# xiangli0608/Creating-2D-laser-slam-from-scratch

Measured on AMD Instinct MI355X. Metric: scan-matches/sec (1081-beam vs 2000x2000 grid), higher is better.
Workload: dtype u8

## Files before the change

### creating-2d-laser-slam-from-scratch_amd/api.py

```python
from __future__ import annotations

import ctypes as C
import os
import sys
import math
import weakref

import numpy as np

from . import build as _build

LSLAM_OK = 0
ERRORS = {
    -1: "LSLAM_ERR_INVALID_ARGUMENT",
    -2: "LSLAM_ERR_NO_DEVICE",
    -3: "LSLAM_ERR_INDEX_OUT_OF_RANGE",
    -4: "LSLAM_ERR_PROBABILITY_SEARCH",
    -5: "LSLAM_ERR_NO_BEST_POSE",
    -6: "LSLAM_ERR_HIP",
    -7: "LSLAM_ERR_SMEAR_DEVIATION",
    -8: "LSLAM_ERR_UNSUPPORTED",
}


# ... 774 lines not shown
    L.lslam_profile_only.argtypes = [vp, C.c_char_p]
    L.lslam_profile_reset.argtypes = [vp]
    L.lslam_profile_read.argtypes = [vp, vp, i32]
    L.lslam_matcher_config_defaults.argtypes = [C.POINTER(MatcherConfig)]
    L.lslam_matcher_config_defaults.restype = None
    L.lslam_matcher_create.argtypes = [vp, C.POINTER(MatcherConfig), C.POINTER(LaserParams), C.POINTER(vp)]
    L.lslam_debug_reduce_lds_bytes.argtypes = [C.POINTER(MatcherConfig), i32, C.POINTER(i32 * 3)]
    L.lslam_debug_reduce_lds_bytes.restype = i32
    L.lslam_matcher_destroy.argtypes = [vp]
    L.lslam_matcher_destroy.restype = None
    L.lslam_matcher_num_beams.argtypes = [vp]
    L.lslam_matcher_grid_info.argtypes = [vp, vp, vp]
    L.lslam_matcher_get_grid_u8.argtypes = [vp, vp]
    L.lslam_matcher_get_kernel_u8.argtypes = [vp, vp]
    L.lslam_matcher_set_grid_u8.argtypes = [vp, vp, vp]
    L.lslam_matcher_set_grid_u8_dev.argtypes = [vp, vp, vp]
    L.lslam_matcher_grid_dev_ptr.restype = vp
    L.lslam_matcher_grid_dev_ptr.argtypes = [vp]
    L.lslam_sensor_pose_from_robot.argtypes = [C.POINTER(LaserParams), vp, vp]
    L.lslam_sensor_pose_from_robot.restype = None
    L.lslam_robot_pose_from_sensor.argtypes = [C.POINTER(LaserParams), vp, vp]
    L.lslam_robot_pose_from_sensor.restype = None
    L.lslam_matcher_set_base_scans.argtypes = [vp, i32, vp, i32, vp, vp]
    L.lslam_matcher_match_scan.argtypes = [vp, i32, vp, i32, vp, vp, vp, i32, i32, vp]
    L.lslam_matcher_match_batch.argtypes = [vp, i32, vp, i32, vp, i32, i32, vp]
    L.lslam_matcher_match_batch_dev_f32.argtypes = [vp, i32, vp, i32, vp, i32, i32, vp]
    L.lslam_matcher_match_batch_dev_f64.argtypes = [vp, i32, vp, i32, vp, i32, i32, vp]
    L.lslam_matcher_debug_lookup_table.argtypes = [vp, vp, vp, dbl, dbl, dbl, vp, C.POINTER(i32)]
    L.lslam_matcher_debug_coarse_sums.argtypes = [vp, vp, vp, vp, C.POINTER(i32), C.POINTER(i32),
                                                  C.POINTER(i32), i32]
    L.lslam_matcher_debug_coarse_sums_batch.argtypes = [vp, i32, vp, i32, vp, vp]
    L.lslam_matcher_debug_fine_sums_batch.argtypes = [vp, i32, vp, i32, vp, vp, vp, C.POINTER(i32), C.POINTER(i32), C.POINTER(i32)]
    L.lslam_matcher_debug_valid_mask.argtypes = [vp, vp, vp, vp, vp]
    L.lslam_frontend_create.argtypes = [vp, i32, dbl, dbl, dbl, C.POINTER(vp)]
    L.lslam_frontend_destroy.argtypes = [vp]
    L.lslam_frontend_destroy.restype = None
    L.lslam_frontend_reset.argtypes = [vp]
    L.lslam_frontend_process.argtypes = [vp, vp, i32, vp, C.POINTER(i32), vp, vp, C.POINTER(dbl)]
    L.lslam_frontend_running_scans.argtypes = [vp]
    L.lslam_frontend_config_defaults.argtypes = [C.POINTER(FrontEndConfig)]
    L.lslam_frontend_config_defaults.restype = None
    L.lslam_frontend_create_ex.argtypes = [vp, C.POINTER(FrontEndConfig), C.POINTER(vp)]
    L.lslam_frontend_process_stamped.argtypes = [vp, vp, i32, vp, dbl, C.POINTER(i32), vp, vp, C.POINTER(dbl)]
    L.lslam_frontend_num_scans.argtypes = [vp]
    L.lslam_frontend_scan_pose.argtypes = [vp, i32, vp]
    L.lslam_frontend_stats.argtypes = [vp, vp]
    L.lslam_frontend_process_many.argtypes = [vp, i32, vp, i32, vp, vp, vp, vp, vp, vp]
    L.lslam_frontend_lookahead_stats.argtypes = [vp, vp]
    L.lslam_frontend_spec_chain_stats.argtypes = [vp, vp]
    L.lslam_debug_frontend_anchor_row.argtypes = [vp, C.c_int, vp]
    L.lslam_occgrid_create_from_scans.argtypes = [vp, C.POINTER(LaserParams), i32, vp, i32, vp, dbl, C.POINTER(vp)]
    L.lslam_occgrid_destroy.argtypes = [vp]
    L.lslam_occgrid_destroy.restype = None
    L.lslam_occgrid_info.argtypes = [vp, vp, vp, C.POINTER(dbl)]
    L.lslam_occgrid_read_u8.argtypes = [vp, vp]
    L.lslam_occgrid_read_ros_i8.argtypes = [vp, vp]
    L.lslam_occgrid_scan_bounds.argtypes = [vp, C.POINTER(LaserParams), i32, vp, i32, vp, vp]
    L.lslam_occgrid_create_partial.argtypes = [vp, C.POINTER(LaserParams), i32, vp, i32, vp, dbl, vp, C.POINTER(vp)]
    L.lslam_occgrid_counter_words.argtypes = [vp, C.POINTER(C.c_size_t)]
    L.lslam_occgrid_export_counters.argtypes = [vp, vp, i32]
    L.lslam_occgrid_import_counters.argtypes = [vp, vp, i32, i32]
    L.lslam_occgrid_counters_dev_ptr.restype = vp
    L.lslam_occgrid_counters_dev_ptr.argtypes = [vp]
    L.lslam_occgrid_ray_cast.argtypes = [vp, i32, vp, vp, dbl, vp]
    L.lslam_occgrid_ray_cast_dev.argtypes = [vp, i32, vp, vp, dbl, vp]
    L.lslam_occgrid_ray_cast_scans.argtypes = [vp, C.POINTER(LaserParams), i32, vp, dbl, vp, i32]
# ... 486 lines not shown
        nx, ny, na = C.c_int(), C.c_int(), C.c_int()
        self.ctx.check(self.L.lslam_matcher_debug_coarse_sums(self.h, r.ctypes.data, p.ctypes.data, None,
                                                              C.byref(nx), C.byref(ny), C.byref(na), 0))
        out = np.zeros((ny.value, nx.value, na.value), dtype=np.int32)
        self.ctx.check(self.L.lslam_matcher_debug_coarse_sums(self.h, r.ctypes.data, p.ctypes.data, out.ctypes.data,
                                                              C.byref(nx), C.byref(ny), C.byref(na),
                                                              int(force_generic)))
        return out

    def coarse_sums_batch(self, ranges, sensor_poses) -> np.ndarray:
        r, p = _f64(ranges), _f64(sensor_poses)
        n = r.shape[0]
        nx, ny, na = C.c_int(), C.c_int(), C.c_int()
        self.ctx.check(self.L.lslam_matcher_debug_coarse_sums(self.h, r.ctypes.data, p.ctypes.data, None,
                                                              C.byref(nx), C.byref(ny), C.byref(na), 0))
        out = np.zeros((n, ny.value, nx.value, na.value), dtype=np.int32)
        self.ctx.check(self.L.lslam_matcher_debug_coarse_sums_batch(self.h, n, r.ctypes.data, r.shape[1], p.ctypes.data,
                                                                    out.ctypes.data))
        return out

    def fine_sums_batch(self, ranges, sensor_poses):
        r, p = _f64(ranges), _f64(sensor_poses)
        n = r.shape[0]
        nx, ny, na = C.c_int(), C.c_int(), C.c_int()
        self.ctx.check(self.L.lslam_matcher_debug_fine_sums_batch(self.h, n, r.ctypes.data, r.shape[1], p.ctypes.data, None, None,
                                                                  C.byref(nx), C.byref(ny), C.byref(na)))
        out = np.zeros((n, ny.value, nx.value, na.value), dtype=np.int32)
        centers = np.zeros((n, 3))
        self.ctx.check(self.L.lslam_matcher_debug_fine_sums_batch(self.h, n, r.ctypes.data, r.shape[1], p.ctypes.data,
                                                                  centers.ctypes.data, out.ctypes.data, C.byref(nx), C.byref(ny),
                                                                  C.byref(na)))
        return out, centers

    def valid_mask(self, ranges, sensor_pose, viewpoint) -> np.ndarray:
        r, p, v = _f64(ranges), _f64(sensor_pose), _f64(viewpoint)
        out = np.zeros(self.num_beams, dtype=np.uint8)
        self.ctx.check(self.L.lslam_matcher_debug_valid_mask(self.h, r.ctypes.data, p.ctypes.data, v.ctypes.data,
                                                             out.ctypes.data))
        return out


class ScanCache:

    PENALIZE, REFINE, QUERY_TAKES_RESULT_POSE = 1, 2, 4

    def __init__(self, ctx: Context, laser: LaserParams):
        self.ctx, self.L = ctx, ctx.L
        h = C.c_void_p()
        ctx.check(self.L.lslam_scan_cache_create(ctx.h, C.byref(laser), C.byref(h)))
        self.h = h
        ctx._adopt(self)

    def close(self):
        if getattr(self, "h", None):
            self.L.lslam_scan_cache_destroy(self.h)
            self.h = None

    def __del__(self):
        try:
            if sys.is_finalizing():
                return
            self.close()
        except Exception:
            pass

    def put(self, scan_id: int, ranges):
# ... 1189 lines not shown
```

### creating-2d-laser-slam-from-scratch_amd/csrc/karto_math.hpp

```cpp
#pragma once

#include <hip/hip_runtime.h>

#include <climits>
#include <cmath>
#include <cstdint>

namespace lslam {

#define LSLAM_HD __host__ __device__ __forceinline__

constexpr double kPi = 3.14159265358979323846;
constexpr double k2Pi = 6.28318530717958647692;
constexpr double kPi180 = 0.01745329251994329577;
constexpr double kTol = 1e-06;
constexpr int32_t kInvalidScan = INT_MAX;
constexpr double kMaxVariance = 500.0;
constexpr double kDistPenaltyGain = 0.2;
constexpr double kAnglePenaltyGain = 0.2;
constexpr int kOccupied = 100;

LSLAM_HD double kround(double v) { return v >= 0.0 ? floor(v + 0.5) : ceil(v - 0.5); }
LSLAM_HD double ksq(double v) { return v * v; }
LSLAM_HD bool double_equal(double a, double b) {
  double d = a - b;
  return d < 0.0 ? d >= -kTol : d <= kTol;
}
LSLAM_HD double normalize_angle(double angle) {
  while (angle < -kPi) {
    if (angle < -k2Pi)
      angle += (uint32_t)(angle / -k2Pi) * k2Pi;
    else
      angle += k2Pi;
  }
  while (angle > kPi) {
    if (angle > k2Pi)
      angle -= (uint32_t)(angle / k2Pi) * k2Pi;
    else
      angle -= k2Pi;
  }
  return angle;
}
LSLAM_HD double normalize_angle_difference(double minuend, double subtrahend) {
  while (minuend - subtrahend < -kPi) minuend += k2Pi;
  while (minuend - subtrahend > kPi) minuend -= k2Pi;
  return minuend;
}
LSLAM_HD int world_to_grid(double w, double offset, double scale) {
  return (int)kround((w - offset) * scale);
}
LSLAM_HD int lattice_count(double offset, double resolution) {
  return (int)(uint32_t)(kround(offset * 2.0 / resolution) + 1);
}

struct Rot2 {
  double m00, m01, m02, m10, m11, m12;
};
LSLAM_HD Rot2 rot_z(double radians) {
  const double x = 0.0, y = 0.0, z = 1.0;
  double c = cos(radians), s = sin(radians), omc = 1.0 - c;
  double xyM = x * y * omc, xzM = x * z * omc, yzM = y * z * omc;
  double xS = x * s, yS = y * s, zS = z * s;
  Rot2 r;
  r.m00 = x * x * omc + c;
  r.m01 = xyM - zS;
  r.m02 = xzM + yS;
  r.m10 = xyM + zS;
  r.m11 = y * y * omc + c;
  r.m12 = yzM - xS;
  return r;
}
LSLAM_HD Rot2 rot_identity() { return Rot2{1.0, 0.0, 0.0, 0.0, 1.0, 0.0}; }
LSLAM_HD void rot_apply(const Rot2& r, double x, double y, double h, double& ox, double& oy) {
  ox = r.m00 * x + r.m01 * y + r.m02 * h;
  oy = r.m10 * x + r.m11 * y + r.m12 * h;
}

struct SensorXform {
  Rot2 rot, inv;
  double tx, ty, th;
};
LSLAM_HD SensorXform sensor_xform(double px, double py, double ph) {
  SensorXform t;
  if (px == 0.0 && py == 0.0 && ph == 0.0) {
    t.rot = rot_identity();
    t.inv = rot_identity();
    t.tx = t.ty = t.th = 0.0;
    return t;
  }
  t.rot = rot_z(ph - 0.0);
  t.inv = rot_z(0.0 - ph);
  t.tx = px;
  t.ty = py;
  t.th = ph - 0.0;
  return t;
}

LSLAM_HD void beam_world_point(double sx, double sy, double sh, double min_angle, double ang_res,
                               uint32_t beam, double r, double& px, double& py) {
  double angle = sh + min_angle + beam * ang_res;
#if defined(__HIP_DEVICE_COMPILE__)
  double sn, cs;
  sincos(angle, &sn, &cs);
  px = sx + (r * cs);
  py = sy + (r * sn);
#else
  px = sx + (r * cos(angle));
  py = sy + (r * sin(angle));
#endif
}

LSLAM_HD void lookup_cell(double lx, double ly, double cosine, double sine, double off_x, double off_y,
                          double scale, int& gx, int& gy) {
  double ox = cosine * lx - sine * ly;
  double oy = sine * lx + cosine * ly;
  gx = world_to_grid(ox + off_x, off_x, scale);
  gy = world_to_grid(oy + off_y, off_y, scale);
}
LSLAM_HD int kround_i32(double v) {
  const int i = (int)(fabs(v) + 0.5);
  return v < 0.0 ? -i : i;
}
LSLAM_HD void lookup_cell_i32(double lx, double ly, double cosine, double sine, double off_x, double off_y,
                              double scale, int& gx, int& gy) {
// ... 111 lines not shown
```

### creating-2d-laser-slam-from-scratch_amd/csrc/scan_matcher.hip

```cpp
#include <algorithm>
#include <atomic>
#include <chrono>
#include <cmath>
#include <cstdlib>
#include <cstring>
#include <type_traits>
#include <vector>

#include "common.hpp"
#include "karto_math.hpp"

using namespace lslam;

#if defined(LSLAM_EXP_SERIAL_PRIO)
#define LSLAM_SERIAL_BEGIN() __builtin_amdgcn_s_setprio(3)
#define LSLAM_SERIAL_END() __builtin_amdgcn_s_setprio(0)
#else
#define LSLAM_SERIAL_BEGIN()
#define LSLAM_SERIAL_END()
#endif

namespace {

LSLAM_STAMP_TABLE(g_sm_stamps)
// ... 31 lines not shown
  if (sc.fast_div) {
    const double q = a * sc.inv_denom;
    return __builtin_fma(__builtin_fma(-q, d, a), sc.inv_denom, q);
  }
  return a / d;
}

constexpr int kTilePad = 512;
constexpr int kTileYOff = 32;
constexpr int kRowZero = 64;
constexpr int kMaxBeamsPerLane = 32;
constexpr int kOccMinScans = 8;
constexpr int kTileMinWaves = 2048;
constexpr int kPipeMinChunk = 256;
constexpr int kMaxGridSide = 32768;

struct Lattice {
  double center[3];
  int gx[kMaxLattice], gy[kMaxLattice];
  int step_x, step_y;
  int status, active;
};

struct CoarseOut {
  double mean[3];
  double cov[9];
  double best;
  int status;
  int expand;
  int flags;
  int pad;
};

__device__ __forceinline__ void pass_setup_wave(int s, int lane, const Geom& g, const PassCfg& pc,
                                                const double* center, int active, Lattice* lat,
                                                double2* cossin, int want_step);

struct PoseArg {
  double v[3];
};
template <typename RT>
__device__ __forceinline__ void scan_prep_block(const RT* __restrict__ ranges, int stride, double sx, double sy, double sh,
                                                const Geom& g, double2* __restrict__ local, double2* __restrict__ world,
                                                const PassCfg& setup_pc, Lattice* setup_lat, double2* setup_cossin,
                                                int setup_step, int bx, int nbx, int s) {
  const int nt = (int)blockDim.x;
  int b = bx * nt + threadIdx.x;
  LSLAM_PHASE_CLOCK(pck);
  __shared__ SensorXform s_t;
  __shared__ double s_h;
  if (local && threadIdx.x == 0) {
    LSLAM_SERIAL_BEGIN();
    s_t = sensor_xform(sx, sy, sh);
    s_h = normalize_angle(0.0 - s_t.th);
    LSLAM_SERIAL_END();
  }
  if (setup_lat && bx == 0 && (int)threadIdx.x >= nt - 64) {
    const double center[3] = {sx, sy, sh};
    pass_setup_wave(s, (int)threadIdx.x - (nt - 64), g, setup_pc, center, 1, setup_lat, setup_cossin, setup_step);
  }
  double r = 0.0, px = 0.0, py = 0.0;
  if (b < g.n_beams) {
    r = (double)ranges[(size_t)s * stride + b];
    beam_world_point(sx, sy, sh, g.min_angle, g.ang_res, (uint32_t)b, r, px, py);
  }
  LSLAM_PHASE_MARK(pck, 0);
  __syncthreads();
  LSLAM_PHASE_MARK(pck, 1);
  for (bool first = true; b < g.n_beams; b += nbx * nt, first = false) {
    if (!first) {
      r = (double)ranges[(size_t)s * stride + b];
      beam_world_point(sx, sy, sh, g.min_angle, g.ang_res, (uint32_t)b, r, px, py);
    }
    size_t o = (size_t)s * g.n_beams + b;
    if (world) world[o] = make_double2(px, py);
    if (local) {
      double lx, ly;
      if (isnan(r) || isinf(r)) {
        lx = ly = __builtin_nan("");
      } else {
        rot_apply(s_t.inv, px - s_t.tx, py - s_t.ty, s_h, lx, ly);
      }
      local[o] = make_double2(lx, ly);
    }
  }
  LSLAM_PHASE_MARK(pck, 2);
  LSLAM_PHASE_FLUSH(pck, g_sm_stamps, 6, (unsigned)(blockIdx.x * (nt >> 6) + (threadIdx.x >> 6)), (threadIdx.x & 63) == 0);
}

template <typename RT>
__global__ void __launch_bounds__(256)
k_scan_prep(const RT* __restrict__ ranges, int stride, const double* __restrict__ poses, Geom g,
            double2* __restrict__ local, double2* __restrict__ world, PassCfg setup_pc, Lattice* setup_lat,
            double2* setup_cossin, int setup_step, PoseArg pose_val) {
  const int s = blockIdx.y;
  const double sx = poses ? poses[3 * s] : pose_val.v[0], sy = poses ? poses[3 * s + 1] : pose_val.v[1],
               sh = poses ? poses[3 * s + 2] : pose_val.v[2];
  scan_prep_block(ranges, stride, sx, sy, sh, g, local, world, setup_pc, setup_lat, setup_cossin, setup_step, (int)blockIdx.x,
                  (int)gridDim.x, s);
}

__device__ __forceinline__ void pass_setup_wave(int s, int lane, const Geom& g, const PassCfg& pc,
                                                const double* center, int active, Lattice* lat,
                                                double2* cossin, int want_step) {
  const double start_x = -pc.off_x, start_y = -pc.off_y;
  auto cell_x = [&](int i) {
    double x = start_x + (uint32_t)i * pc.res_x;
    double npx = center[0] + x;
    return world_to_grid(npx, g.off_x, g.scale) + g.border;
  };
  auto cell_y = [&](int j) {
    double y = start_y + (uint32_t)j * pc.res_y;
    double npy = center[1] + y;
    return world_to_grid(npy, g.off_y, g.scale) + g.border;
  };
  const int stx0 = pc.nx > 1 ? cell_x(1) - cell_x(0) : want_step;
  const int sty0 = pc.ny > 1 ? cell_y(1) - cell_y(0) : want_step;
  bool out_of_range = false, uneven_x = false, uneven_y = false;
  Lattice& L = lat[s];
  for (int i = lane; i < kMaxLattice; i += 64) {
    int cx = 0, cy = 0;
    if (i < pc.nx) {
      cx = cell_x(i);
      out_of_range |= cx < 0 || cx >= g.width;
      if (i >= 1) uneven_x |= cx - cell_x(i - 1) != stx0;
    }
    if (i < pc.ny) {
      cy = cell_y(i);
      out_of_range |= cy < 0 || cy >= g.height;
      if (i >= 1) uneven_y |= cy - cell_y(i - 1) != sty0;
    }
    L.gx[i] = cx;
    L.gy[i] = cy;
  }
  for (int a = lane; a < pc.na; a += 64) {
    const double angle = (center[2] - pc.ang_off) + (uint32_t)a * pc.ang_res;
    cossin[(size_t)s * kMaxAngles + a] = make_double2(cos(angle), sin(angle));
  }
  const int status = __any(out_of_range) ? LSLAM_ERR_INDEX_OUT_OF_RANGE : 0;
  const int stx = __any(uneven_x) ? 0 : stx0, sty = __any(uneven_y) ? 0 : sty0;
  if (lane == 0) {
    L.center[0] = center[0]; L.center[1] = center[1]; L.center[2] = center[2];
    L.step_x = stx;
    L.step_y = sty;
    L.status = status;
    L.active = active;
  }
}

__global__ void __launch_bounds__(64)
k_pass_setup(int S, Geom g, PassCfg pc, const double* __restrict__ poses, const CoarseOut* __restrict__ coarse,
             Lattice* __restrict__ lat, double2* __restrict__ cossin, int want_step) {
  const int s = blockIdx.x;
  if (s >= S) return;
  double center[3];
  int active = 1;
  if (pc.mode == 0) {
    center[0] = poses[3 * s]; center[1] = poses[3 * s + 1]; center[2] = poses[3 * s + 2];
  } else if (pc.mode == 1) {
    center[0] = poses[3 * s]; center[1] = poses[3 * s + 1]; center[2] = poses[3 * s + 2];
    active = coarse[s].expand && coarse[s].status == 0;
  } else {
    center[0] = coarse[s].mean[0]; center[1] = coarse[s].mean[1]; center[2] = coarse[s].mean[2];
    active = coarse[s].status == 0;
  }
  pass_setup_wave(s, threadIdx.x, g, pc, center, active, lat, cossin, want_step);
}

__global__ void __launch_bounds__(256)
k_deinterleave(const uint8_t* __restrict__ grid, uint8_t* __restrict__ f0, uint8_t* __restrict__ f1, int n8) {
  int t = blockIdx.x * blockDim.x + threadIdx.x;
  if (t >= n8) return;
  uint2 v = ((const uint2*)grid)[t];
  uint32_t e = (v.x & 0xFFu) | ((v.x >> 8) & 0xFF00u) | ((v.y & 0xFFu) << 16) | ((v.y << 8) & 0xFF000000u);
  uint32_t o = ((v.x >> 8) & 0xFFu) | ((v.x >> 16) & 0xFF00u) | ((v.y << 8) & 0xFF0000u) | (v.y & 0xFF000000u);
  ((uint32_t*)f0)[t] = e;
  ((uint32_t*)f1)[t] = o;
}

// ... 970 lines not shown
  cd.angle = (center[2] - pc.ang_off) + (uint32_t)a * pc.ang_res;
  return cd;
}

__device__ __forceinline__ double penalized(int32_t sum, const Cand& cd, const double* center, int n_beams,
                                            const SearchCfg& sc) {
  double r = response_of_sum(sum, n_beams, sc);
  if (sc.do_penalize && !double_equal(r, 0.0)) {
    double sd = ksq(cd.x) + ksq(cd.y);
    double dp = 1.0 - (kDistPenaltyGain * sd / sc.dvp);
    dp = dp > sc.min_dp ? dp : sc.min_dp;
    double sad = ksq(cd.angle - center[2]);
    double ap = 1.0 - (kAnglePenaltyGain * sad / sc.avp);
    ap = ap > sc.min_ap ? ap : sc.min_ap;
    r *= (dp * ap);
  }
  return r;
}

__device__ __forceinline__ double block_max(double v, double* sh, int tid, int nthreads) {
#pragma unroll
  for (int m = 1; m < 64; m <<= 1) {
    const double o = __shfl_xor(v, m);
    v = v > o ? v : o;
  }
  if ((tid & 63) == 0) sh[tid >> 6] = v;
  __syncthreads();
  double r = sh[0];
  for (int w = 1; w < (nthreads >> 6); w++) r = r > sh[w] ? r : sh[w];
  __syncthreads();
  return r;
}

__device__ int tie_average(const uint32_t* mask, int total, const PassCfg& pc, const double* center,
                           double* avg) {
  double ax = 0, ay = 0, tx = 0, ty = 0;
  int cnt = 0;
  int words = (total + 31) / 32;
  for (int wd = 0; wd < words; wd++) {
    uint32_t m = mask[wd];
    while (m) {
      int bit = __ffs(m) - 1;
      m &= m - 1;
      int k = wd * 32 + bit;
      Cand cd = cand_of(k, pc, center);
      double h = normalize_angle(cd.angle);
      ax += center[0] + cd.x;
      ay += center[1] + cd.y;
      double sn, cs;
      sincos(h, &sn, &cs);
      tx += cs;
      ty += sn;
      cnt++;
    }
  }
  if (cnt == 0) return 0;
  ax /= cnt; ay /= cnt; tx /= cnt; ty /= cnt;
  avg[0] = ax; avg[1] = ay; avg[2] = atan2(ty, tx);
  return cnt;
}

template <bool CACHE>
__global__ void __launch_bounds__(256)
k_reduce_coarse(Geom g, PassCfg pc, SearchCfg sc, const Lattice* __restrict__ lat,
                int32_t* resp, size_t resp_stride, CoarseOut* __restrict__ out,
                int use_expansion, int pass_index, const uint8_t* __restrict__ grid,
                const double2* __restrict__ local, int fb_step) {
  extern __shared__ __align__(16) unsigned char smem[];
// ... 265 lines not shown
        while (nzw) {
          const int wd = wv * 64 + (__ffsll((long long)nzw) - 1);
          nzw &= nzw - 1;
          uint32_t m = mask[wd];
          while (m) {
            const int bit = __ffs(m) - 1;
            m &= m - 1;
            const Cand cd = cand_of(wd * 32 + bit, pc, center);
            const double h = normalize_angle(cd.angle);
            ax += center[0] + cd.x;
            ay += center[1] + cd.y;
            double sn, cs;
            sincos(h, &sn, &cs);
            tx += cs;
            ty += sn;
            cnt++;
          }
        }
      }
      if (cnt == 0) {
        st = LSLAM_ERR_NO_BEST_POSE;
      } else {
        ax /= cnt; ay /= cnt; tx /= cnt; ty /= cnt;
        avg[0] = ax; avg[1] = ay; avg[2] = atan2(ty, tx);
      }
    }
    s_avg[0] = avg[0]; s_avg[1] = avg[1]; s_avg[2] = avg[2];
    s_status = st;
    LSLAM_SERIAL_END();
  }
  __syncthreads();
  LSLAM_PHASE_MARK(pck, 4);
  if (fine_cossin != nullptr && tid >= NT - 64) {
    const double center2[3] = {s_avg[0], s_avg[1], s_avg[2]};
    pass_setup_wave(s, tid - (NT - 64), g, fine_pc, center2, s_status == 0, lat, fine_cossin, fine_step);
  }
  const double dx = s_avg[0] - center[0], dy = s_avg[1] - center[1];
  const double thr = s_best - 0.1;
  int n_pass = 0;
  for (int c0 = 0; c0 < ncand; c0 += NT) {
    const int c = c0 + tid;
    double rr = 0.0, t1 = 0.0, t2 = 0.0, t3 = 0.0;
    bool pass = false;
    if (c < ncand) {
      const int xi = c % pc.nx, yi = c / pc.nx;
      const double x = -pc.off_x + (uint32_t)xi * pc.res_x;
      const double y = -pc.off_y + (uint32_t)yi * pc.res_y;
      rr = cell[c] >= 0 ? probs[cell[c]] : 0.0;
      t1 = (ksq(x - dx) * rr);
      t2 = ((x - dx) * (y - dy) * rr);
      t3 = (ksq(y - dy) * rr);
      pass = rr >= thr;
    }
    const unsigned long long bal = __ballot(pass);
    if ((tid & 63) == 0) s_wcnt[tid >> 6] = __popcll(bal);
    __syncthreads();
    int off = n_pass;
    for (int w = 0; w < (tid >> 6); w++) off += s_wcnt[w];
    for (int w = 0; w < (NT + 63) / 64; w++) n_pass += s_wcnt[w];
    if (pass) {
      const int k = off + __popcll(bal & ((1ull << (tid & 63)) - 1ull));
      terms[4 * k + 0] = rr; terms[4 * k + 1] = t1; terms[4 * k + 2] = t2; terms[4 * k + 3] = t3;
    }
    __syncthreads();
  }
  LSLAM_PHASE_MARK(pck, 5);
  if (tid == 0) {
    CoarseOut o;
// ... 633 lines not shown
    }
  };
  __shared__ double s_avg[3];
  __shared__ double s_best;
  __shared__ int s_status, s_pos;
  uint32_t* mask = (uint32_t*)smem;
  const CoarseOut& co = coarse[s];
  if (!do_refine || co.status != 0) {
    if (tid == 0) {
      lslam_match_result res;
      for (int i = 0; i < 3; i++) res.pose[i] = co.status ? 0.0 : co.mean[i];
      for (int i = 0; i < 9; i++) res.covariance[i] = co.status ? 0.0 : co.cov[i];
      res.response = co.status ? 0.0 : co.best;
      res.status = co.status;
      res.flags = co.flags;
      out[s] = res;
      signal_done();
    }
    return;
  }
  const Lattice& L = lat[s];
  if (L.status != 0) {
    if (tid == 0) {
      lslam_match_result res;
      memset(&res, 0, sizeof res);
      res.status = L.status;
      res.flags = co.flags;
      out[s] = res;
      signal_done();
    }
    return;
  }
  LSLAM_PHASE_CLOCK(pck);
  block_generic_fallback(grid, g, pc, L, local + (size_t)s * g.n_beams, r, fb_step, tid, NT);
  const int ncand = pc.nx * pc.ny;
  const int total = ncand * pc.na;
  const double center[3] = {L.center[0], L.center[1], L.center[2]};
  constexpr int kKeep = 4;
  double mine[kKeep];
  auto value = [&](int k) -> double {
    const int a = k % pc.na, c = k / pc.na;
    return penalized(r[a * ncand + c], cand_of(k, pc, center), center, g.n_beams, sc);
  };
  double lm = -1.0;
#pragma unroll
  for (int i = 0; i < kKeep; i++) {
    const int k = tid + NT * i;
    mine[i] = k < total ? value(k) : -1.0;
    lm = lm > mine[i] ? lm : mine[i];
  }
  for (int k = tid + NT * kKeep; k < total; k += NT) {
    const double v = value(k);
    lm = lm > v ? lm : v;
  }
  const int words = (total + 31) / 32;
  for (int wd = tid; wd < words; wd += NT) mask[wd] = 0u;
  for (int a = tid; a < kMaxAngles; a += NT) asum[a] = 0;
  LSLAM_PHASE_MARK(pck, 0);
  const double best = block_max(lm, sh, tid, NT);
  LSLAM_PHASE_MARK(pck, 1);
#pragma unroll
  for (int i = 0; i < kKeep; i++) {
    const int k = tid + NT * i;
    if (k < total && double_equal(mine[i], best)) atomicOr(&mask[k >> 5], 1u << (k & 31));
  }
  for (int k = tid + NT * kKeep; k < total; k += NT)
    if (double_equal(value(k), best)) atomicOr(&mask[k >> 5], 1u << (k & 31));
  __syncthreads();
  if (tid == 0) {
    LSLAM_SERIAL_BEGIN();
    double avg[3] = {0, 0, 0};
    int st = 0;
    if (tie_average(mask, total, pc, center, avg) == 0) st = LSLAM_ERR_NO_BEST_POSE;
    int pos = 0;
    if (st == 0) {
      int gx = world_to_grid(avg[0], g.off_x, g.scale) + g.border;
      int gy = world_to_grid(avg[1], g.off_y, g.scale) + g.border;
      if (gx < 0 || gx >= g.width || gy < 0 || gy >= g.height) st = LSLAM_ERR_INDEX_OUT_OF_RANGE;
      pos = gx + gy * g.stride;
    }
    s_avg[0] = avg[0]; s_avg[1] = avg[1]; s_avg[2] = avg[2];
    s_best = best;
    s_status = st;
    s_pos = pos;
    LSLAM_SERIAL_END();
  }
  __syncthreads();
  LSLAM_PHASE_MARK(pck, 2);
  if (s_status == 0) {
    int hit = -1;
    for (int yi = 0, c = 0; yi < pc.ny; yi++) {
      const int row = L.gy[yi] * g.stride;
      for (int xi = 0; xi < pc.nx; xi++, c++)
        if (L.gx[xi] + row == s_pos) hit = c;
    }
    if (hit >= 0) {
      for (int a = tid; a < pc.na; a += NT) asum[a] = r[a * ncand + hit];
    } else {
      const double2* lp = local + (size_t)s * g.n_beams;
      const int pos = s_pos;
      for (int a = 0; a < pc.na; a++) {
        double angle = (center[2] - pc.ang_off) + (uint32_t)a * pc.ang_res;
        double cosine = cos(angle), sine = sin(angle);
        int32_t part = 0;
        for (int b = tid; b < g.n_beams; b += NT) {
          double2 p = lp[b];
          if (isnan(p.x)) continue;
          int t = lookup_offset(p.x, p.y, cosine, sine, g.off_x, g.off_y, g.scale, g.stride);
          long long idx = (long long)pos + t;
          if (idx >= 0 && idx < g.data_size) part += grid[idx];
        }
        for (int o = 32; o > 0; o >>= 1) part += __shfl_xor(part, o);
        if ((tid & 63) == 0) atomicAdd(&asum[a], part);
      }
    }
  }
  __syncthreads();
  LSLAM_PHASE_MARK(pck, 3);
  LSLAM_PHASE_FLUSH(pck, g_sm_stamps, 4, (unsigned)(s * (NT >> 6) + (tid >> 6)), (tid & 63) == 0 && tid != 0);
  if (tid != 0) return;
  LSLAM_SERIAL_BEGIN();
  lslam_match_result res;
  memset(&res, 0, sizeof res);
  res.flags = co.flags;
  res.status = s_status;
  if (s_status == 0) {
    double bestAngle = normalize_angle_difference(s_avg[2], center[2]);
    double norm = 0.0, acc = 0.0;
    double start = center[2] - pc.ang_off;
    for (int a = 0; a < pc.na; a++) {
      double angle = start + (uint32_t)a * pc.ang_res;
      double rr = response_of_sum(asum[a], g.n_beams, sc);
      if (rr >= (s_best - 0.1)) {
        norm += rr;
        acc += (ksq(angle - bestAngle) * rr);
      }
    }
    if (norm > kTol) {
      if (acc < kTol) acc = ksq(pc.ang_res);
      acc /= norm;
    } else {
      acc = 1000 * ksq(pc.ang_res);
    }
    for (int i = 0; i < 9; i++) res.covariance[i] = co.cov[i];
    res.covariance[8] = acc;
    res.pose[0] = s_avg[0]; res.pose[1] = s_avg[1]; res.pose[2] = s_avg[2];
    res.response = s_best > 1.0 ? 1.0 : s_best;
  }
  out[s] = res;
  signal_done();
  LSLAM_PHASE_MARK(pck, 4);
  LSLAM_PHASE_FLUSH(pck, g_sm_stamps, 4, (unsigned)(s * (NT >> 6)), true);
}

template <int NT>
__global__ void __launch_bounds__(NT)
k_reduce_fine(const uint8_t* __restrict__ grid, Geom g, PassCfg pc, SearchCfg sc,
              const Lattice* __restrict__ lat, int32_t* resp, size_t resp_stride,
              const double2* __restrict__ local, const CoarseOut* __restrict__ coarse,
              lslam_match_result* __restrict__ out, int do_refine, int fb_step, int* done_flag, int done_ticket) {
  extern __shared__ __align__(16) unsigned char smem[];
  reduce_fine_block<NT>((int)blockIdx.x, (int)threadIdx.x, grid, g, pc, sc, lat, resp + (size_t)blockIdx.x * resp_stride, local,
                        coarse, out, do_refine, fb_step, done_flag, done_ticket, smem);
}

constexpr int kStepFineAngles = 4;
template <int NXD>
constexpr int step_wave_area() { return rows_wave_area<NXD>(); }
// ... 680 lines not shown
__global__ void k_add_scans_serial(int B, int n, const double2* __restrict__ world, int ring_start, int cap,
                                   const uint8_t* __restrict__ valid, Geom g,
                                   const uint8_t* __restrict__ kernel, uint8_t* __restrict__ grid) {
  if (blockIdx.x || threadIdx.x) return;
  const int hk = g.kernel_size / 2;
  for (int i = 0; i < B * n; i++) {
    if (!valid[i]) continue;
    const double2 wp = world[(size_t)((ring_start + i / n) % cap) * n + (i % n)];
    int gx, gy;
    if (!base_point_cell(wp, g, gx, gy)) continue;
    size_t idx = (size_t)(gx + g.border) + (size_t)(gy + g.border) * g.stride;
    if (grid[idx] == kOccupied) continue;
    grid[idx] = kOccupied;
    for (int j = -hk; j <= hk; j++) {
      uint8_t* row = grid + (size_t)(gx + g.border) + (size_t)(gy + j + g.border) * g.stride;
      for (int k = -hk; k <= hk; k++) {
        uint8_t kv = kernel[(k + hk) + g.kernel_size * (j + hk)];
        if (kv > row[k]) row[k] = kv;
      }
    }
  }
}

__global__ void k_debug_table(Geom g, const double2* __restrict__ local, double angle_center,
                              double angle_offset, double angle_res, int na, int32_t* __restrict__ out) {
  int b = blockIdx.x * blockDim.x + threadIdx.x;
  int a = blockIdx.y;
  if (b >= g.n_beams || a >= na) return;
  double angle = (angle_center - angle_offset) + (uint32_t)a * angle_res;
  double2 p = local[b];
  int32_t v = kInvalidScan;
  if (!isnan(p.x)) v = lookup_offset(p.x, p.y, cos(angle), sin(angle), g.off_x, g.off_y, g.scale, g.stride);
  out[(size_t)a * g.n_beams + b] = v;
}

}

struct lslam_matcher {
  lslam_context* ctx = nullptr;
  lslam_matcher_config cfg;
  lslam_laser laser;
  Geom g;
  std::vector<uint8_t> h_kernel;
  bool kernel_center_only = true;
  uint8_t* d_grid_alloc = nullptr;
  uint8_t* d_grid = nullptr;
  uint8_t* d_marks_alloc = nullptr;
  uint8_t* d_marks = nullptr;
  int mark_epoch = 0;
  uint8_t* d_kernel = nullptr;
  uint8_t* d_sub_alloc = nullptr;
  uint8_t* d_sub[2] = {nullptr, nullptr};
  bool sub_dirty = true;
  bool occ_dirty = true;
  std::atomic<bool> busy{false};
  bool use_row_occupancy = true;
  bool collect_stats = false;
  bool lds_staged = false;
  int rows_waves = 1;
  bool rows_mfma = true;
  bool grid_fits_i8 = true;
  int64_t rows_mfma_launches = 0;
  bool fine_mfma = true;
  int64_t fine_mfma_launches = 0;
  SpecArgs spec_req{};
  bool spec_armed = false, spec_launched = false;
// ... 1450 lines not shown
  rc = match_batch_impl<double>(m, 1, m->d_query.p, n, m->d_qpose.p, do_penalize, do_refine, m->h_result, nullptr, 0);
  if (rc) return rc;
  rc = wait_record(m);
  if (rc) return rc;
  *out = *m->h_result;
  return LSLAM_OK;
}

int lslam_matcher_debug_lookup_table(lslam_matcher* m, const double* ranges, const double pose[3],
                                     double angle_center, double angle_offset, double angle_res,
                                     int32_t* out, int* n_angles_out) {
  if (!m || !ranges || !pose || !n_angles_out) return LSLAM_ERR_INVALID_ARGUMENT;
  lslam_context* ctx = m->ctx;
  const Geom g = m->g;
  int na = n_angles_of(angle_offset, angle_res);
  *n_angles_out = na;
  if (!out || g.n_beams == 0) return LSLAM_OK;
  int rc = pipe_join(m);
  if (rc) return rc;
  rc = upload_scans(m, 1, ranges, g.n_beams, pose);
  if (rc) return rc;
  LSLAM_HIP(ctx, m->d_local.reserve((size_t)g.n_beams));
  LSLAM_HIP(ctx, m->d_dbg.reserve((size_t)na * g.n_beams));
  launch(ctx, "scan_prep", k_scan_prep<double>, dim3((g.n_beams + 255) / 256, 1), dim3(256), 0,
         (const double*)m->d_ranges64.p, g.n_beams, (const double*)m->d_poses.p, g, m->d_local.p, (double2*)nullptr, PassCfg{}, (Lattice*)nullptr, (double2*)nullptr, 0, PoseArg{});
  launch(ctx, "debug_table", k_debug_table, dim3((g.n_beams + 255) / 256, na), dim3(256), 0, g,
         (const double2*)m->d_local.p, angle_center, angle_offset, angle_res, na, m->d_dbg.p);
  LSLAM_HIP(ctx, hipMemcpyAsync(out, m->d_dbg.p, (size_t)na * g.n_beams * sizeof(int32_t), hipMemcpyDeviceToHost,
                                ctx->stream));
  LSLAM_HIP(ctx, hipStreamSynchronize(ctx->stream));
  return LSLAM_OK;
}

int lslam_matcher_debug_coarse_sums(lslam_matcher* m, const double* ranges, const double pose[3], int32_t* out,
                                    int* nx, int* ny, int* na, int force_generic) {
  if (!m || !ranges || !pose) return LSLAM_ERR_INVALID_ARGUMENT;
  lslam_context* ctx = m->ctx;
  const Geom g = m->g;
  const double res = 1.0 / g.scale;
  double off = 0.5 * ((double)g.probs_side - 1) * res;
  int lx = lattice_count(off, 2 * res);
  int la = n_angles_of(m->cfg.coarse_search_angle_offset, m->cfg.coarse_angle_resolution);
  if (nx) *nx = lx;
  if (ny) *ny = lx;
  if (na) *na = la;
  if (!out || g.n_beams == 0) return LSLAM_OK;
  int rc = upload_scans(m, 1, ranges, g.n_beams, pose);
  if (rc) return rc;
  LSLAM_HIP(ctx, m->d_results.reserve(1));
  LSLAM_HIP(ctx, m->d_dbg.reserve((size_t)lx * lx * la));
  rc = match_batch_impl<double>(m, 1, m->d_ranges64.p, g.n_beams, m->d_poses.p, 1, 0, m->d_results.p, m->d_dbg.p,
                                force_generic);
  if (rc) return rc;
  std::vector<int32_t> tmp((size_t)lx * lx * la);
  LSLAM_HIP(ctx, hipMemcpyAsync(tmp.data(), m->d_dbg.p, tmp.size() * sizeof(int32_t), hipMemcpyDeviceToHost,
                                ctx->stream));
  LSLAM_HIP(ctx, hipStreamSynchronize(ctx->stream));
  const int ncand = lx * lx;
  for (int a = 0; a < la; a++)
    for (int c = 0; c < ncand; c++) out[(size_t)c * la + a] = tmp[(size_t)a * ncand + c];
  return LSLAM_OK;
}

int lslam_matcher_debug_coarse_sums_batch(lslam_matcher* m, int n_scans, const double* ranges, int ranges_stride,
                                          const double* poses, int32_t* out) {
  if (!m || !ranges || !poses || !out || n_scans <= 0) return LSLAM_ERR_INVALID_ARGUMENT;
// ... 108 lines not shown
```

### include/lslam_gpu.h

```cpp
#ifndef LSLAM_GPU_H
#define LSLAM_GPU_H

#include <stddef.h>
#include <stdint.h>

#ifdef __cplusplus
extern "C" {
#endif

#define LSLAM_ABI_VERSION 5

typedef enum lslam_status {
  LSLAM_OK = 0,
  LSLAM_ERR_INVALID_ARGUMENT = -1,
  LSLAM_ERR_NO_DEVICE = -2,
  LSLAM_ERR_INDEX_OUT_OF_RANGE = -3,
  LSLAM_ERR_PROBABILITY_SEARCH = -4,
  LSLAM_ERR_NO_BEST_POSE = -5,
  LSLAM_ERR_HIP = -6,
  LSLAM_ERR_SMEAR_DEVIATION = -7,
  LSLAM_ERR_UNSUPPORTED = -8,
  LSLAM_ERR_NO_DATA = -9
} lslam_status;

// ... 111 lines not shown
                                      int do_penalize, int do_refine,
                                      lslam_match_result* out_dev);

typedef struct lslam_scan_cache lslam_scan_cache;
int lslam_scan_cache_create(lslam_context* ctx, const lslam_laser* laser, lslam_scan_cache** out);
void lslam_scan_cache_destroy(lslam_scan_cache* cache);
int lslam_scan_cache_put(lslam_scan_cache* cache, int64_t scan_id, const double* ranges);
int lslam_scan_cache_contains(const lslam_scan_cache* cache, int64_t scan_id);
int lslam_scan_cache_forget(lslam_scan_cache* cache, int64_t scan_id);
int lslam_scan_cache_size(const lslam_scan_cache* cache);
int lslam_scan_cache_prepare(lslam_scan_cache* cache, int64_t scan_id, const double sensor_pose[3]);
int lslam_scan_cache_counters(const lslam_scan_cache* cache, int64_t out[5]);
enum {
  LSLAM_MATCH_PENALIZE = 1,
  LSLAM_MATCH_REFINE = 2,
  LSLAM_MATCH_QUERY_TAKES_RESULT_POSE = 4
};
int lslam_matcher_match_scan_cached(lslam_matcher* m, lslam_scan_cache* cache, int n_base, const int64_t* base_ids,
                                    const double* base_sensor_poses, int64_t query_id, const double* query_ranges,
                                    const double query_sensor_pose[3], int flags, lslam_match_result* out);

int lslam_matcher_debug_lookup_table(lslam_matcher* m, const double* ranges,
                                     const double sensor_pose[3], double angle_center,
                                     double angle_offset, double angle_resolution,
                                     int32_t* out_host, int* n_angles_out);
int lslam_matcher_debug_coarse_sums(lslam_matcher* m, const double* ranges,
                                    const double sensor_pose[3], int32_t* out_host, int* nx,
                                    int* ny, int* na, int force_generic_kernel);
int lslam_matcher_debug_coarse_sums_batch(lslam_matcher* m, int n_scans, const double* ranges, int ranges_stride,
                                          const double* sensor_poses, int32_t* out);
int lslam_matcher_debug_fine_sums_batch(lslam_matcher* m, int n_scans, const double* ranges, int ranges_stride,
                                        const double* sensor_poses, double* centers_out, int32_t* out, int* nx, int* ny,
                                        int* na);
int lslam_matcher_debug_valid_mask(lslam_matcher* m, const double* ranges,
                                   const double sensor_pose[3], const double viewpoint[2],
                                   uint8_t* out_host);

typedef struct lslam_pool lslam_pool;
int lslam_pool_create(int n_devices, const lslam_matcher_config* cfg, const lslam_laser* laser, lslam_pool** out);
int lslam_pool_create_on(const int* devices, int n_devices, const lslam_matcher_config* cfg, const lslam_laser* laser,
                         lslam_pool** out);
void lslam_pool_destroy(lslam_pool* pool);
int lslam_pool_devices(const lslam_pool* pool);
lslam_matcher* lslam_pool_matcher(lslam_pool* pool, int i);
const char* lslam_pool_last_error(const lslam_pool* pool);
int lslam_pool_set_base_scans(lslam_pool* pool, int n_scans, const double* ranges, int ranges_stride,
                              const double* sensor_poses, const double center_pose[3], int replicate_by_rebuild);
int lslam_pool_match_batch(lslam_pool* pool, int n_scans, const double* ranges, int ranges_stride,
                           const double* sensor_poses, int do_penalize, int do_refine, lslam_match_result* out);

typedef struct lslam_frontend lslam_frontend;
typedef struct lslam_frontend_config {
  int32_t scan_buffer_size;
  int32_t use_scan_barycenter;
  int32_t do_loop_closing;
  int32_t loop_match_minimum_chain_size;
  double scan_buffer_maximum_scan_distance;
  double minimum_travel_distance;
  double minimum_travel_heading;
  double minimum_time_interval;
  double link_match_minimum_response_fine;
  double link_scan_maximum_distance;
  double loop_search_maximum_distance;
  double loop_match_maximum_variance_coarse;
  double loop_match_minimum_response_coarse;
  double loop_match_minimum_response_fine;
// ... 468 lines not shown
```

Measured before the change: 8.100 million.

## Parallelize setup trig, lattice checks, fine penalty tables and angle variance terms

Moves the sensor-transform sin/cos from a single serial thread into the setup wave using sincos with shuffles, and rewrites the lattice step/bounds check to use wave shuffles instead of recomputing neighbour cells. The fine pass now precomputes per-cell and per-angle penalty factors in shared memory, walks candidate indices incrementally instead of using div/mod, and computes angular variance terms in parallel before thread 0 sums them. A debug sincos entry point is added. These changes aim to cut serial double-precision work on the critical path, at the cost of extra shared-memory use and syncs, and possible tiny numeric differences from table multiplication order.

```diff
diff --git a/creating-2d-laser-slam-from-scratch_amd/api.py b/creating-2d-laser-slam-from-scratch_amd/api.py
--- a/creating-2d-laser-slam-from-scratch_amd/api.py
+++ b/creating-2d-laser-slam-from-scratch_amd/api.py
@@ -830,6 +830,8 @@
     L.lslam_matcher_debug_coarse_sums_batch.argtypes = [vp, i32, vp, i32, vp, vp]
     L.lslam_matcher_debug_fine_sums_batch.argtypes = [vp, i32, vp, i32, vp, vp, vp, C.POINTER(i32), C.POINTER(i32), C.POINTER(i32)]
     L.lslam_matcher_debug_valid_mask.argtypes = [vp, vp, vp, vp, vp]
+    if hasattr(L, "lslam_matcher_debug_sincos"):
+        L.lslam_matcher_debug_sincos.argtypes = [vp, vp, i32, vp]
     L.lslam_frontend_create.argtypes = [vp, i32, dbl, dbl, dbl, C.POINTER(vp)]
     L.lslam_frontend_destroy.argtypes = [vp]
     L.lslam_frontend_destroy.restype = None
@@ -1382,6 +1384,12 @@
                                                                   C.byref(na)))
         return out, centers
 
+    def debug_sincos(self, x) -> np.ndarray:
+        v = _f64(x).reshape(-1)
+        out = np.zeros((len(v), 4))
+        self.ctx.check(self.L.lslam_matcher_debug_sincos(self.h, v.ctypes.data, len(v), out.ctypes.data))
+        return out
+
     def valid_mask(self, ranges, sensor_pose, viewpoint) -> np.ndarray:
         r, p, v = _f64(ranges), _f64(sensor_pose), _f64(viewpoint)
         out = np.zeros(self.num_beams, dtype=np.uint8)
diff --git a/creating-2d-laser-slam-from-scratch_amd/csrc/karto_math.hpp b/creating-2d-laser-slam-from-scratch_amd/csrc/karto_math.hpp
--- a/creating-2d-laser-slam-from-scratch_amd/csrc/karto_math.hpp
+++ b/creating-2d-laser-slam-from-scratch_amd/csrc/karto_math.hpp
@@ -56,9 +56,9 @@
 struct Rot2 {
   double m00, m01, m02, m10, m11, m12;
 };
-LSLAM_HD Rot2 rot_z(double radians) {
+LSLAM_HD Rot2 rot_z_cs(double c, double s) {
   const double x = 0.0, y = 0.0, z = 1.0;
-  double c = cos(radians), s = sin(radians), omc = 1.0 - c;
+  double omc = 1.0 - c;
   double xyM = x * y * omc, xzM = x * z * omc, yzM = y * z * omc;
   double xS = x * s, yS = y * s, zS = z * s;
   Rot2 r;
@@ -69,6 +69,10 @@
   r.m11 = y * y * omc + c;
   r.m12 = yzM - xS;
   return r;
+}
+LSLAM_HD Rot2 rot_z(double radians) {
+  double c = cos(radians), s = sin(radians);
+  return rot_z_cs(c, s);
 }
 LSLAM_HD Rot2 rot_identity() { return Rot2{1.0, 0.0, 0.0, 0.0, 1.0, 0.0}; }
 LSLAM_HD void rot_apply(const Rot2& r, double x, double y, double h, double& ox, double& oy) {
@@ -90,6 +94,21 @@
   }
   t.rot = rot_z(ph - 0.0);
   t.inv = rot_z(0.0 - ph);
+  t.tx = px;
+  t.ty = py;
+  t.th = ph - 0.0;
+  return t;
+}
+LSLAM_HD SensorXform sensor_xform_cs(double px, double py, double ph, double c_rot, double s_rot, double c_inv, double s_inv) {
+  SensorXform t;
+  if (px == 0.0 && py == 0.0 && ph == 0.0) {
+    t.rot = rot_identity();
+    t.inv = rot_identity();
+    t.tx = t.ty = t.th = 0.0;
+    return t;
+  }
+  t.rot = rot_z_cs(c_rot, s_rot);
+  t.inv = rot_z_cs(c_inv, s_inv);
   t.tx = px;
   t.ty = py;
   t.th = ph - 0.0;
diff --git a/creating-2d-laser-slam-from-scratch_amd/csrc/scan_matcher.hip b/creating-2d-laser-slam-from-scratch_amd/csrc/scan_matcher.hip
--- a/creating-2d-laser-slam-from-scratch_amd/csrc/scan_matcher.hip
+++ b/creating-2d-laser-slam-from-scratch_amd/csrc/scan_matcher.hip
@@ -87,9 +87,12 @@
   int pad;
 };
 
+template <bool with_angles = true>
 __device__ __forceinline__ void pass_setup_wave(int s, int lane, const Geom& g, const PassCfg& pc,
                                                 const double* center, int active, Lattice* lat,
                                                 double2* cossin, int want_step);
+__device__ __forceinline__ double2 setup_trig_wave(int s, int lane, const PassCfg& pc, double heading, int na,
+                                                   double2* cossin, int n_extra, double extra0, double extra1);
 
 struct PoseArg {
   double v[3];
@@ -104,15 +107,26 @@
   LSLAM_PHASE_CLOCK(pck);
   __shared__ SensorXform s_t;
   __shared__ double s_h;
-  if (local && threadIdx.x == 0) {
-    LSLAM_SERIAL_BEGIN();
-    s_t = sensor_xform(sx, sy, sh);
-    s_h = normalize_angle(0.0 - s_t.th);
-    LSLAM_SERIAL_END();
-  }
-  if (setup_lat && bx == 0 && (int)threadIdx.x >= nt - 64) {
-    const double center[3] = {sx, sy, sh};
-    pass_setup_wave(s, (int)threadIdx.x - (nt - 64), g, setup_pc, center, 1, setup_lat, setup_cossin, setup_step);
+  const bool do_setup = setup_lat && bx == 0;
+  if ((int)threadIdx.x >= nt - 64 && (do_setup || local)) {
+    const int lane = (int)threadIdx.x - (nt - 64);
+    if (do_setup) {
+      const double center[3] = {sx, sy, sh};
+      pass_setup_wave<false>(s, lane, g, setup_pc, center, 1, setup_lat, setup_cossin, setup_step);
+    }
+    const int na = do_setup ? setup_pc.na : 0;
+    const double2 cs = setup_trig_wave(s, lane, setup_pc, sh, na, setup_cossin, local ? 2 : 0, sh - 0.0, 0.0 - sh);
+    if (local) {
+      const int l_rot = na & 63, l_inv = (na + 1) & 63;
+      const double c_rot = __shfl(cs.x, l_rot), s_rot = __shfl(cs.y, l_rot);
+      const double c_inv = __shfl(cs.x, l_inv), s_inv = __shfl(cs.y, l_inv);
+      if (lane == 0) {
+        LSLAM_SERIAL_BEGIN();
+        s_t = sensor_xform_cs(sx, sy, sh, c_rot, s_rot, c_inv, s_inv);
+        s_h = normalize_angle(0.0 - s_t.th);
+        LSLAM_SERIAL_END();
+      }
+    }
   }
   double r = 0.0, px = 0.0, py = 0.0;
   if (b < g.n_beams) {
@@ -155,6 +169,21 @@
                   (int)gridDim.x, s);
 }
 
+__device__ __forceinline__ double2 setup_trig_wave(int s, int lane, const PassCfg& pc, double heading, int na,
+                                                   double2* cossin, int n_extra, double extra0, double extra1) {
+  double2 mine = make_double2(0.0, 0.0);
+  const double start = heading - pc.ang_off;
+  for (int a = lane; a < na + n_extra; a += 64) {
+    const double angle = a < na ? start + (uint32_t)a * pc.ang_res : (a == na ? extra0 : extra1);
+    double sn, cs;
+    sincos(angle, &sn, &cs);
+    if (a < na) cossin[(size_t)s * kMaxAngles + a] = make_double2(cs, sn);
+    else mine = make_double2(cs, sn);
+  }
+  return mine;
+}
+
+template <bool with_angles>
 __device__ __forceinline__ void pass_setup_wave(int s, int lane, const Geom& g, const PassCfg& pc,
                                                 const double* center, int active, Lattice* lat,
                                                 double2* cossin, int want_step) {
@@ -169,37 +198,52 @@
     double npy = center[1] + y;
     return world_to_grid(npy, g.off_y, g.scale) + g.border;
   };
-  const int stx0 = pc.nx > 1 ? cell_x(1) - cell_x(0) : want_step;
-  const int sty0 = pc.ny > 1 ? cell_y(1) - cell_y(0) : want_step;
+  int stx0 = want_step, sty0 = want_step, carry_x = 0, carry_y = 0;
+  const int n_side = pc.nx > pc.ny ? pc.nx : pc.ny;
   bool out_of_range = false, uneven_x = false, uneven_y = false;
   Lattice& L = lat[s];
-  for (int i = lane; i < kMaxLattice; i += 64) {
+  if (lane == 0) {
+    L.center[0] = center[0]; L.center[1] = center[1]; L.center[2] = center[2];
+    L.active = active;
+  }
+#pragma unroll 1
+  for (int i0 = 0; i0 < kMaxLattice; i0 += 64) {
+    const int i = i0 + lane;
     int cx = 0, cy = 0;
-    if (i < pc.nx) {
-      cx = cell_x(i);
-      out_of_range |= cx < 0 || cx >= g.width;
-      if (i >= 1) uneven_x |= cx - cell_x(i - 1) != stx0;
-    }
-    if (i < pc.ny) {
-      cy = cell_y(i);
-      out_of_range |= cy < 0 || cy >= g.height;
-      if (i >= 1) uneven_y |= cy - cell_y(i - 1) != sty0;
+    if (i0 < n_side) {
+      if (i < pc.nx) cx = cell_x(i);
+      if (i < pc.ny) cy = cell_y(i);
+      int bx = __shfl_up(cx, 1), by = __shfl_up(cy, 1);
+      if (lane == 0) { bx = carry_x; by = carry_y; }
+      const int dx = cx - bx, dy = cy - by;
+      if (i0 == 0) {
+        if (pc.nx > 1) stx0 = __builtin_amdgcn_readlane(dx, 1);
+        if (pc.ny > 1) sty0 = __builtin_amdgcn_readlane(dy, 1);
+      }
+      if (i < pc.nx) {
+        out_of_range |= cx < 0 || cx >= g.width;
+        if (i >= 1) uneven_x |= dx != stx0;
+      }
+      if (i < pc.ny) {
+        out_of_range |= cy < 0 || cy >= g.height;
+        if (i >= 1) uneven_y |= dy != sty0;
+      }
+      carry_x = __builtin_amdgcn_readlane(cx, 63);
+      carry_y = __builtin_amdgcn_readlane(cy, 63);
     }
     L.gx[i] = cx;
     L.gy[i] = cy;
-  }
-  for (int a = lane; a < pc.na; a += 64) {
-    const double angle = (center[2] - pc.ang_off) + (uint32_t)a * pc.ang_res;
-    cossin[(size_t)s * kMaxAngles + a] = make_double2(cos(angle), sin(angle));
   }
   const int status = __any(out_of_range) ? LSLAM_ERR_INDEX_OUT_OF_RANGE : 0;
   const int stx = __any(uneven_x) ? 0 : stx0, sty = __any(uneven_y) ? 0 : sty0;
   if (lane == 0) {
-    L.center[0] = center[0]; L.center[1] = center[1]; L.center[2] = center[2];
     L.step_x = stx;
     L.step_y = sty;
     L.status = status;
-    L.active = active;
+  }
+  if (with_angles) {
+    asm volatile("" ::: "memory");
+    setup_trig_wave(s, lane, pc, center[2], pc.na, cossin, 0, 0.0, 0.0);
   }
 }
 
@@ -1236,8 +1280,8 @@
   return r;
 }
 
-__device__ int tie_average(const uint32_t* mask, int total, const PassCfg& pc, const double* center,
-                           double* avg) {
+__device__ __forceinline__ int tie_average(const uint32_t* mask, int total, const PassCfg& pc, const double* center,
+                                           double* avg) {
   double ax = 0, ay = 0, tx = 0, ty = 0;
   int cnt = 0;
   int words = (total + 31) / 32;
@@ -1569,8 +1613,7 @@
   __syncthreads();
   LSLAM_PHASE_MARK(pck, 4);
   if (fine_cossin != nullptr && tid >= NT - 64) {
-    const double center2[3] = {s_avg[0], s_avg[1], s_avg[2]};
-    pass_setup_wave(s, tid - (NT - 64), g, fine_pc, center2, s_status == 0, lat, fine_cossin, fine_step);
+    pass_setup_wave(s, tid - (NT - 64), g, fine_pc, s_avg, s_status == 0, lat, fine_cossin, fine_step);
   }
   const double dx = s_avg[0] - center[0], dy = s_avg[1] - center[1];
   const double thr = s_best - 0.1;
@@ -2270,25 +2313,65 @@
     return;
   }
   LSLAM_PHASE_CLOCK(pck);
-  block_generic_fallback(grid, g, pc, L, local + (size_t)s * g.n_beams, r, fb_step, tid, NT);
+  block_generic_fallback<kReduceNarrowChunk>(grid, g, pc, L, local + (size_t)s * g.n_beams, r, fb_step, tid, NT);
   const int ncand = pc.nx * pc.ny;
   const int total = ncand * pc.na;
   const double center[3] = {L.center[0], L.center[1], L.center[2]};
   constexpr int kKeep = 4;
   double mine[kKeep];
-  auto value = [&](int k) -> double {
-    const int a = k % pc.na, c = k / pc.na;
-    return penalized(r[a * ncand + c], cand_of(k, pc, center), center, g.n_beams, sc);
+#if !defined(LSLAM_TUNE_FINE_TABLES)
+#define LSLAM_TUNE_FINE_TABLES 1
+#endif
+  constexpr int kTabAt = 16;
+  double* tab = sh + kTabAt;
+  const bool tabulated = LSLAM_TUNE_FINE_TABLES && ncand + pc.na <= NT - kTabAt;
+  if (tabulated && sc.do_penalize) {
+    if (tid < ncand + pc.na) {
+      const bool is_cell = tid < ncand;
+      double q;
+      if (is_cell) {
+        const int xi = tid % pc.nx, yi = tid / pc.nx;
+        const double x = -pc.off_x + (uint32_t)xi * pc.res_x;
+        const double y = -pc.off_y + (uint32_t)yi * pc.res_y;
+        q = ksq(x) + ksq(y);
+      } else {
+        const double angle = (center[2] - pc.ang_off) + (uint32_t)(tid - ncand) * pc.ang_res;
+        q = ksq(angle - center[2]);
+      }
+      const double p = 1.0 - ((is_cell ? kDistPenaltyGain : kAnglePenaltyGain) * q / (is_cell ? sc.dvp : sc.avp));
+      const double lo = is_cell ? sc.min_dp : sc.min_ap;
+      tab[tid] = p > lo ? p : lo;
+    }
+    __syncthreads();
+  }
+  const int step_c = NT / pc.na, step_a = NT % pc.na;
+  struct At {
+    int c, a;
   };
+  auto advance = [&](At& at) {
+    at.c += step_c;
+    at.a += step_a;
+    if (at.a >= pc.na) { at.a -= pc.na; at.c++; }
+  };
+  auto value = [&](int k, const At& at) -> double {
+    const int32_t sum = r[at.a * ncand + at.c];
+    if (!tabulated) return penalized(sum, cand_of(k, pc, center), center, g.n_beams, sc);
+    double v = response_of_sum(sum, g.n_beams, sc);
+    if (sc.do_penalize && !double_equal(v, 0.0)) v *= (tab[at.c] * tab[ncand + at.a]);
+    return v;
+  };
+  At at{tid / pc.na, tid % pc.na};
   double lm = -1.0;
 #pragma unroll
   for (int i = 0; i < kKeep; i++) {
     const int k = tid + NT * i;
-    mine[i] = k < total ? value(k) : -1.0;
+    mine[i] = k < total ? value(k, at) : -1.0;
     lm = lm > mine[i] ? lm : mine[i];
-  }
-  for (int k = tid + NT * kKeep; k < total; k += NT) {
-    const double v = value(k);
+    advance(at);
+  }
+  const At at_rest = at;
+  for (int k = tid + NT * kKeep; k < total; k += NT, advance(at)) {
+    const double v = value(k, at);
     lm = lm > v ? lm : v;
   }
   const int words = (total + 31) / 32;
@@ -2302,8 +2385,9 @@
     const int k = tid + NT * i;
     if (k < total && double_equal(mine[i], best)) atomicOr(&mask[k >> 5], 1u << (k & 31));
   }
-  for (int k = tid + NT * kKeep; k < total; k += NT)
-    if (double_equal(value(k), best)) atomicOr(&mask[k >> 5], 1u << (k & 31));
+  at = at_rest;
+  for (int k = tid + NT * kKeep; k < total; k += NT, advance(at))
+    if (double_equal(value(k, at), best)) atomicOr(&mask[k >> 5], 1u << (k & 31));
   __syncthreads();
   if (tid == 0) {
     LSLAM_SERIAL_BEGIN();
@@ -2354,6 +2438,18 @@
     }
   }
   __syncthreads();
+  const bool terms_by_lane = LSLAM_TUNE_FINE_TABLES && 2 * pc.na <= NT - kTabAt;
+  if (terms_by_lane && s_status == 0) {
+    const double bestAngle = normalize_angle_difference(s_avg[2], center[2]);
+    const double start = center[2] - pc.ang_off;
+    for (int a = tid; a < pc.na; a += NT) {
+      const double angle = start + (uint32_t)a * pc.ang_res;
+      const double rr = response_of_sum(asum[a], g.n_beams, sc);
+      tab[2 * a] = rr;
+      tab[2 * a + 1] = (ksq(angle - bestAngle) * rr);
+    }
+    __syncthreads();
+  }
   LSLAM_PHASE_MARK(pck, 3);
   LSLAM_PHASE_FLUSH(pck, g_sm_stamps, 4, (unsigned)(s * (NT >> 6) + (tid >> 6)), (tid & 63) == 0 && tid != 0);
   if (tid != 0) return;
@@ -2363,15 +2459,25 @@
   res.flags = co.flags;
   res.status = s_status;
   if (s_status == 0) {
-    double bestAngle = normalize_angle_difference(s_avg[2], center[2]);
     double norm = 0.0, acc = 0.0;
-    double start = center[2] - pc.ang_off;
-    for (int a = 0; a < pc.na; a++) {
-      double angle = start + (uint32_t)a * pc.ang_res;
-      double rr = response_of_sum(asum[a], g.n_beams, sc);
-      if (rr >= (s_best - 0.1)) {
-        norm += rr;
-        acc += (ksq(angle - bestAngle) * rr);
+    if (terms_by_lane) {
+      for (int a = 0; a < pc.na; a++) {
+        const double rr = tab[2 * a];
+        if (rr >= (s_best - 0.1)) {
+          norm += rr;
+          acc += tab[2 * a + 1];
+        }
+      }
+    } else {
+      double bestAngle = normalize_angle_difference(s_avg[2], center[2]);
+      double start = center[2] - pc.ang_off;
+      for (int a = 0; a < pc.na; a++) {
+        double angle = start + (uint32_t)a * pc.ang_res;
+        double rr = response_of_sum(asum[a], g.n_beams, sc);
+        if (rr >= (s_best - 0.1)) {
+          norm += rr;
+          acc += (ksq(angle - bestAngle) * rr);
+        }
       }
     }
     if (norm > kTol) {
@@ -3118,6 +3224,18 @@
   int32_t v = kInvalidScan;
   if (!isnan(p.x)) v = lookup_offset(p.x, p.y, cos(angle), sin(angle), g.off_x, g.off_y, g.scale, g.stride);
   out[(size_t)a * g.n_beams + b] = v;
+}
+
+__global__ void k_debug_sincos(const double* __restrict__ x, int n, double* __restrict__ out) {
+  const int i = blockIdx.x * blockDim.x + threadIdx.x;
+  if (i >= n) return;
+  const double v = x[i];
+  double sn, cs;
+  sincos(v, &sn, &cs);
+  out[4 * (size_t)i + 0] = sin(v);
+  out[4 * (size_t)i + 1] = cos(v);
+  out[4 * (size_t)i + 2] = sn;
+  out[4 * (size_t)i + 3] = cs;
 }
 
 }
@@ -4634,6 +4752,22 @@
   return LSLAM_OK;
 }
 
+int lslam_matcher_debug_sincos(lslam_matcher* m, const double* x, int n, double* out) {
+  if (!m || !x || !out || n < 0) return LSLAM_ERR_INVALID_ARGUMENT;
+  if (n == 0) return LSLAM_OK;
+  lslam_context* ctx = m->ctx;
+  int rc = pipe_join(m);
+  if (rc) return rc;
+  LSLAM_HIP(ctx, m->d_dbg.reserve((size_t)n * 10));
+  double* d_x = (double*)m->d_dbg.p;
+  double* d_out = d_x + n;
+  LSLAM_HIP(ctx, hipMemcpyAsync(d_x, x, (size_t)n * sizeof(double), hipMemcpyHostToDevice, ctx->stream));
+  launch(ctx, "debug_sincos", k_debug_sincos, dim3((n + 255) / 256), dim3(256), 0, (const double*)d_x, n, d_out);
+  LSLAM_HIP(ctx, hipMemcpyAsync(out, d_out, (size_t)n * 4 * sizeof(double), hipMemcpyDeviceToHost, ctx->stream));
+  LSLAM_HIP(ctx, hipStreamSynchronize(ctx->stream));
+  return LSLAM_OK;
+}
+
 int lslam_matcher_debug_coarse_sums(lslam_matcher* m, const double* ranges, const double pose[3], int32_t* out,
                                     int* nx, int* ny, int* na, int force_generic) {
   if (!m || !ranges || !pose) return LSLAM_ERR_INVALID_ARGUMENT;
diff --git a/include/lslam_gpu.h b/include/lslam_gpu.h
--- a/include/lslam_gpu.h
+++ b/include/lslam_gpu.h
@@ -167,6 +167,7 @@
 int lslam_matcher_debug_fine_sums_batch(lslam_matcher* m, int n_scans, const double* ranges, int ranges_stride,
                                         const double* sensor_poses, double* centers_out, int32_t* out, int* nx, int* ny,
                                         int* na);
+int lslam_matcher_debug_sincos(lslam_matcher* m, const double* x, int n, double* out_host);
 int lslam_matcher_debug_valid_mask(lslam_matcher* m, const double* ranges,
                                    const double sensor_pose[3], const double viewpoint[2],
                                    uint8_t* out_host);
```

New measurement: 8.171 million (median of 6 runs). Within noise of the previous version (+0.9%).
